# exanauts/SqpSolver.jl

Hardware: AMD Instinct MI355X
Metric: QP subproblems/sec on batched ACOPF; fp64 KKT LDL^T TFLOPS vs MFMA peak (higher is better)
Workload: dtype f64

## Files before the change

### sqpsolver.jl_amd/csrc/mfront.hip

```cpp
#include "ctx.hpp"
#include "dev_util.hpp"
#include "mf_dev.hpp"
#include <cstdlib>
#include <mutex>

namespace sqphip {

#ifdef SQPHIP_MF_TRACE
__device__ long long g_mf_trace[1 << 16][8];
#define MF_TR(i) if (inst == 0 && threadIdx.x == 0 && s < (1 << 16)) g_mf_trace[s][i] = (long long)wall_clock64();
__device__ long long g_mf_trace2[1 << 12][16];
#define MF_TRW(i) if (W == 0 && trs >= 0 && trs < (1 << 12) && lane == 0) g_mf_trace2[trs][i] = (long long)clock64();
__device__ long long g_mf_trace3[1 << 12][16];
#define MF_TRS(i) if (inst == 0 && tid == 0 && s < (1 << 12)) g_mf_trace3[s][i] = (long long)clock64();
#define MF_TR2S(a, b) if (inst == 0 && lane == 0 && j < 64 && wave < 2) g_mf_trace3[(do_fwd ? 64 : 0) + j][wave == 0 ? (a) : (b)] = (long long)clock64();
#define MF_TR2W(c) if (trj >= 0 && lane == 0) g_mf_trace3[trj][c] = (long long)clock64();
#define MF_TRSP(c) if (inst == 0 && cand == 0 && tid == 0 && k < 64) g_mf_trace3[128 + k][c] = (long long)wall_clock64();
#else
#define MF_TR(i)
#define MF_TRW(i)
#define MF_TRS(i)
#define MF_TR2S(a, b)
#define MF_TR2W(c)
#define MF_TRSP(c)
// ... 333 lines not shown
                    acc[q] = __builtin_amdgcn_mfma_f64_16x16x4f64(a, b, acc[q], 0, 0, 0);
                }
        }
    }
    __syncthreads();
    MF_TR(4)
    double *dinv = mf_dinv(d, inst, cand) + f0, *vv = mf_vv(d, inst, cand) + f0;
#pragma unroll
    for (int q = 0; q < MAXT; ++q) {
        if (ti_[q] < 0) continue;
#pragma unroll
        for (int rr = 0; rr < 4; ++rr) {
            const int col = 16 * tj_[q] + l4 + 4 * rr, row = 16 * ti_[q] + l15;
            const double v = acc[q][rr];
            if (col < nc) {
                if (row > col && row < fs) G[(long)col * ld + row] = v * dl[col];
                else if (row == fs && with_rhs) vv[col] = v * dl[col];
            } else if (col < fs && row >= col && row <= fs) G[(long)col * ld + row] = v;
        }
    }
    for (int k = tid; k < nc; k += NT) dinv[k] = dl[k];
    MF_TR(5)
}

struct MfBlk4 { double i0, i1, i2, i3, m10, m20, m21, m30, m31, m32; };

__device__ __forceinline__ MfBlk4 mf_ldl4(double a00, double a10, double a11, double a20, double a21, double a22, double a30,
                                           double a31, double a32, double a33, int bw)
{
    double i1 = 0.0, i2 = 0.0, i3 = 0.0, l21 = 0.0, l31 = 0.0, l32 = 0.0;
    const double i0 = mf_rcp(a00);
    const double l10 = a10 * i0, l20 = a20 * i0, l30 = a30 * i0;
#if SQPHIP_MF_LDL4_FAST
    {
        const double p11 = a10 * a10, p21 = a10 * a20, p22 = a20 * a20, p31 = a10 * a30, p32 = a20 * a30, p33 = a30 * a30;
        a11 = fma(-p11, i0, a11); a21 = fma(-p21, i0, a21); a22 = fma(-p22, i0, a22); a31 = fma(-p31, i0, a31); a32 = fma(-p32, i0, a32); a33 = fma(-p33, i0, a33);
    }
    if (bw > 1) {
        i1 = mf_rcp(a11); l21 = a21 * i1; l31 = a31 * i1;
        const double q22 = a21 * a21, q32 = a21 * a31, q33 = a31 * a31;
        a22 = fma(-q22, i1, a22); a32 = fma(-q32, i1, a32); a33 = fma(-q33, i1, a33);
    }
    if (bw > 2) { i2 = mf_rcp(a22); l32 = a32 * i2; a33 = fma(-(a32 * a32), i2, a33); }
#else
    a11 -= l10 * a10; a21 -= l10 * a20; a22 -= l20 * a20; a31 -= l10 * a30; a32 -= l20 * a30; a33 -= l30 * a30;
    if (bw > 1) { i1 = mf_rcp(a11); l21 = a21 * i1; l31 = a31 * i1; a22 -= l21 * a21; a32 -= l21 * a31; a33 -= l31 * a31; }
    if (bw > 2) { i2 = mf_rcp(a22); l32 = a32 * i2; a33 -= l32 * a32; }
#endif
    if (bw > 3) i3 = mf_rcp(a33);
    MfBlk4 B;
    B.i0 = i0; B.i1 = i1; B.i2 = i2; B.i3 = i3;
    B.m10 = -l10; B.m21 = -l21; B.m32 = -l32;
    B.m20 = -(l20 + l21 * B.m10);
    B.m31 = -(l31 + l32 * B.m21);
    B.m30 = -(l30 + l31 * B.m10 + l32 * B.m20);
    return B;
}

struct MfLaneSel { double s0, s1, s2, s3; };
__device__ __forceinline__ MfLaneSel mf_lane_sel(int l4)
{
    return {l4 == 0 ? 1.0 : 0.0, l4 == 1 ? 1.0 : 0.0, l4 == 2 ? 1.0 : 0.0, l4 == 3 ? 1.0 : 0.0};
}
__device__ __forceinline__ double mf_sel_ic(const MfLaneSel &S, const MfBlk4 &B)
{
    return fma(S.s3, B.i3, fma(S.s2, B.i2, fma(S.s1, B.i1, S.s0 * B.i0)));
}
__device__ __forceinline__ double mf_apply4(double x, int l15, const MfLaneSel &S, const MfBlk4 &B)
{
    const MfRows V = mf_rows3(x, l15);
    const double v0 = V.r0, v1 = V.r1, v2 = V.r2;
    const double c0 = fma(S.s3, B.m30, fma(S.s2, B.m20, S.s1 * B.m10));
    const double c1 = fma(S.s3, B.m31, S.s2 * B.m21);
    const double c2 = S.s3 * B.m32;
    return fma(c2, v2, fma(c1, v1, fma(c0, v0, x)));
}

__device__ __forceinline__ void wave_sync_lds()
{
    __builtin_amdgcn_fence(__ATOMIC_ACQ_REL, "wavefront");
    __builtin_amdgcn_wave_barrier();
}

__host__ __device__ constexpr int mf_front_lds_doubles(int T, int NW, bool ldsimg)
{
    const int R = 16 * T, u = (ldsimg ? R * R : 0) > 16 * R ? R * R : 16 * R;
    return u + 256 + 40 + R + 64 * NW;
}

template <int T, int NW, int W> struct MfTileSet {
    static constexpr int NROWS = W < T ? (T - W + NW - 1) / NW : 0;
    static constexpr int NTILES = NROWS > 0 ? NROWS * (2 * W + (NROWS - 1) * NW + 2) / 2 : 1;
};

template <int T, int NW, int W> struct MfAcc { d4 v[MfTileSet<T, NW, W>::NTILES]; };

template <int T, int NW, int W, bool LDSIMG>
__device__ __forceinline__ void mf_front_load(MfAcc<T, NW, W> &A, const double *F, int LD, int fs, int lane)
{
    auto &acc = A.v;
    constexpr int NROWS = MfTileSet<T, NW, W>::NROWS;
    const int l15 = lane & 15, l4 = lane >> 4;
    int o = 0;
#pragma unroll
    for (int s = 0; s < NROWS; ++s) {
        const int ti = W + s * NW;
#pragma unroll
        for (int tj = 0; tj <= ti; ++tj)
#pragma unroll
            for (int rr = 0; rr < 4; ++rr) {
                const int col = 16 * tj + l4 + 4 * rr, row = 16 * ti + l15;
                const bool in = LDSIMG || (row <= fs && col < fs);
                acc[o + tj][rr] = in ? F[col * LD + row] : 0.0;
            }
        o += ti + 1;
    }
}

__device__ __forceinline__ void lds_barrier()
{
    asm volatile("s_waitcnt lgkmcnt(0)\n\ts_barrier" ::: "memory");
}
template <bool LDSBAR> __device__ __forceinline__ void mf_elim_barrier() { if constexpr (LDSBAR) lds_barrier(); else __syncthreads(); }

template <int T, int NW, int W, bool LDSIMG>
__device__ __forceinline__ void mf_front_store_col(const MfAcc<T, NW, W> &A, int tk, double *G, int ld, int fs, int nc, int with_rhs,
                                                   const double *lds, double *vv, int lane)
{
    const auto &acc = A.v;
    constexpr int R = 16 * T;
    constexpr int U = (LDSIMG ? R * R : 0) > 16 * R ? R * R : 16 * R;
    constexpr int NROWS = MfTileSet<T, NW, W>::NROWS;
    const double *dl = lds + U + 256 + 40;
    const int l15 = lane & 15, l4 = lane >> 4;
    int o = 0;
#pragma unroll
    for (int s = 0; s < NROWS; ++s) {
        const int ti = W + s * NW;
        if (ti >= tk) {
            const bool inside = ti > tk && 16 * ti + 15 < fs;
            if (inside && 16 * tk + 15 < nc) {
#pragma unroll
                for (int rr = 0; rr < 4; ++rr) {
                    const int col = 16 * tk + l4 + 4 * rr;
                    G[(long)col * ld + 16 * ti + l15] = acc[o + tk][rr] * dl[col];
                }
            } else {
#pragma unroll
                for (int rr = 0; rr < 4; ++rr) {
                    const int col = 16 * tk + l4 + 4 * rr, row = 16 * ti + l15;
                    const double v = acc[o + tk][rr];
                    if (col < nc) {
                        if (row > col && row < fs) G[(long)col * ld + row] = v * dl[col];
                        else if (row == fs && with_rhs) vv[col] = v * dl[col];
                    }
                }
            }
        }
        o += ti + 1;
    }
}

template <int T, int NW, int W, bool LDSIMG, bool LDSBAR = false, bool EARLY = false>
__device__ __forceinline__ void mf_front_elim(MfAcc<T, NW, W> &A, int nc, double *lds, int lane, int trs, double *G = nullptr, int ld = 0,
                                              int fs = 0, int with_rhs = 0, double *vv = nullptr)
{
    auto &acc = A.v;
    constexpr int R = 16 * T;
    constexpr int U = (LDSIMG ? R * R : 0) > 16 * R ? R * R : 16 * R;
    constexpr int NROWS = MfTileSet<T, NW, W>::NROWS;
    double *Lp = lds, *dtile = lds + U, *rec = dtile + 256, *dl = rec + 40, *dsc = dl + R + 64 * W;
    const int l15 = lane & 15, l4 = lane >> 4;
    const MfLaneSel LS = mf_lane_sel(l4);
#pragma unroll
    for (int tk = 0; tk < T; ++tk) {
        if (16 * tk >= nc) break;
        if (tk == 1) { MF_TRW(9) }
        const int live = nc - 16 * tk;
        if (tk % NW == W) {
            constexpr int dummy = 0; (void)dummy;
            const int sd = (tk - W) / NW;
            const int od = sd * (2 * W + (sd - 1) * NW + 2) / 2 + tk;
            d4 dt = acc[od];
            d4 ls = {0.0, 0.0, 0.0, 0.0};
#pragma unroll
            for (int sub = 0; sub < 4; ++sub) {
                if (4 * sub >= live) break;
                const int bw = live - 4 * sub < 4 ? live - 4 * sub : 4, b0 = 4 * sub;
                const double dv = dt[sub];
#if SQPHIP_MF_SHFL
                dsc[lane] = dv;
                wave_sync_lds();
                if (tk == 0 && sub == 0) { MF_TRW(11) }
                const double a00 = dsc[b0], a10 = dsc[b0 + 1], a11 = dsc[b0 + 17], a20 = dsc[b0 + 2], a21 = dsc[b0 + 18],
                             a22 = dsc[b0 + 34], a30 = dsc[b0 + 3], a31 = dsc[b0 + 19], a32 = dsc[b0 + 35], a33 = dsc[b0 + 51];
                wave_sync_lds();
#else
                if (tk == 0 && sub == 0) { MF_TRW(11) }
                const double a00 = mf_readlane(dv, b0), a10 = mf_readlane(dv, b0 + 1), a11 = mf_readlane(dv, b0 + 17),
                             a20 = mf_readlane(dv, b0 + 2), a21 = mf_readlane(dv, b0 + 18), a22 = mf_readlane(dv, b0 + 34),
                             a30 = mf_readlane(dv, b0 + 3), a31 = mf_readlane(dv, b0 + 19), a32 = mf_readlane(dv, b0 + 35),
                             a33 = mf_readlane(dv, b0 + 51);
#endif
#ifdef SQPHIP_MF_TRACE
                if (tk == 0 && sub == 0) { asm volatile("s_waitcnt lgkmcnt(0)" ::: "memory"); MF_TRW(12) }
#endif
                const MfBlk4 B = mf_ldl4(a00, a10, a11, a20, a21, a22, a30, a31, a32, a33, bw);
#ifdef SQPHIP_MF_TRACE
                if (tk == 0 && sub == 0) { double tdep = B.m30; asm volatile("v_mov_b64 %0, %0" : "+v"(tdep)); MF_TRW(13) }
#endif
                const double x = mf_apply4(dv, l15, LS, B);
                const double ic = mf_sel_ic(LS, B);
                dt[sub] = x;
                ls[sub] = x * ic;
#ifdef SQPHIP_MF_TRACE
                if (tk == 0 && sub == 0) { double tdep = ls[sub]; asm volatile("v_mov_b64 %0, %0" : "+v"(tdep)); MF_TRW(14) }
#endif
                dt = __builtin_amdgcn_mfma_f64_16x16x4f64(l15 >= b0 + 4 ? -ls[sub] : 0.0, x, dt, 0, 0, 0);
#ifdef SQPHIP_MF_TRACE
                if (tk == 0 && sub == 0) { double tdep = dt[1]; asm volatile("v_mov_b64 %0, %0" : "+v"(tdep)); MF_TRW(15) }
#endif
                if (lane == 0) {
                    double *o = rec + 10 * sub;
                    o[0] = B.i0; o[1] = B.i1; o[2] = B.i2; o[3] = B.i3; o[4] = B.m10; o[5] = B.m20; o[6] = B.m21; o[7] = B.m30;
                    o[8] = B.m31; o[9] = B.m32;
                }
                if (l15 == 0 && l4 < bw) dl[16 * tk + b0 + l4] = ic;
            }
#pragma unroll
            for (int sub = 0; sub < 4; ++sub) dtile[64 * sub + lane] = ls[sub];
            acc[od] = dt;
        }
        if (tk == 0) { MF_TRW(3) }
        mf_elim_barrier<LDSBAR || EARLY>();
        if (tk == 0) { MF_TRW(4) }
        {
            int o = 0;
#pragma unroll
            for (int s = 0; s < NROWS; ++s) {
                const int ti = W + s * NW;
                if (ti > tk) {
                    d4 pt = acc[o + tk];
#pragma unroll
                    for (int sub = 0; sub < 4; ++sub) {
                        if (4 * sub >= live) break;
                        const double *q = rec + 10 * sub;
                        MfBlk4 B;
                        B.i0 = q[0]; B.i1 = q[1]; B.i2 = q[2]; B.i3 = q[3]; B.m10 = q[4]; B.m20 = q[5]; B.m21 = q[6]; B.m30 = q[7];
                        B.m31 = q[8]; B.m32 = q[9];
                        const double x = mf_apply4(pt[sub], l15, LS, B);
                        const double ic = mf_sel_ic(LS, B);
                        pt[sub] = x;
                        Lp[(4 * sub + l4) * R + 16 * ti + l15] = x * ic;
                        if (sub < 3) pt = __builtin_amdgcn_mfma_f64_16x16x4f64(l15 >= 4 * sub + 4 ? -dtile[64 * sub + lane] : 0.0, x, pt, 0, 0, 0);
                    }
                    acc[o + tk] = pt;
                }
                o += ti + 1;
            }
        }
        if (tk == 0) { MF_TRW(5) }
        mf_elim_barrier<LDSBAR || EARLY>();
        if (tk == 0) { MF_TRW(6) }
        {
            int o = 0;
#pragma unroll
            for (int s = 0; s < NROWS; ++s) {
                const int ti = W + s * NW;
                if (ti > tk) {
                    const d4 xr = acc[o + tk];
#pragma unroll
                    for (int tj = tk + 1; tj <= ti; ++tj)
#pragma unroll
                        for (int sub = 0; sub < 4; ++sub) {
                            if (4 * sub >= live) break;
                            acc[o + tj] = __builtin_amdgcn_mfma_f64_16x16x4f64(-Lp[(4 * sub + l4) * R + 16 * tj + l15], xr[sub], acc[o + tj], 0, 0, 0);
                        }
                }
                o += ti + 1;
            }
        }
        if constexpr (EARLY) mf_front_store_col<T, NW, W, LDSIMG>(A, tk, G, ld, fs, nc, with_rhs, lds, vv, lane);
    }
}

template <int T, int NW, int W, bool LDSIMG, bool EARLY = false>
__device__ __forceinline__ void mf_front_store(const MfAcc<T, NW, W> &A, double *G, int ld, int fs, int nc,
                                               int with_rhs, double *CB, int ldcb, const double *lds, double *dinv, double *vv, int lane)
{
    const auto &acc = A.v;
    constexpr int R = 16 * T;
    constexpr int U = (LDSIMG ? R * R : 0) > 16 * R ? R * R : 16 * R;
    constexpr int NROWS = MfTileSet<T, NW, W>::NROWS;
    const double *dl = lds + U + 256 + 40;
    const int l15 = lane & 15, l4 = lane >> 4;
    int o = 0;
#pragma unroll
    for (int s = 0; s < NROWS; ++s) {
        const int ti = W + s * NW;
#pragma unroll
        for (int tj = 0; tj <= ti; ++tj) {
            const bool inside = ti > tj && 16 * ti + 15 < fs;
            if (inside && 16 * tj + 15 < nc) {
                if constexpr (!EARLY) {
#pragma unroll
                    for (int rr = 0; rr < 4; ++rr) {
                        const int col = 16 * tj + l4 + 4 * rr;
                        G[(long)col * ld + 16 * ti + l15] = acc[o + tj][rr] * dl[col];
                    }
                }
            } else if (inside && 16 * tj >= nc) {
#pragma unroll
                for (int rr = 0; rr < 4; ++rr) CB[(long)(16 * tj + l4 + 4 * rr) * ldcb + 16 * ti + l15] = acc[o + tj][rr];
            } else {
#pragma unroll
                for (int rr = 0; rr < 4; ++rr) {
                    const int col = 16 * tj + l4 + 4 * rr, row = 16 * ti + l15;
                    const double v = acc[o + tj][rr];
                    if (col < nc) {
                        if constexpr (!EARLY) {
                            if (row > col && row < fs) G[(long)col * ld + row] = v * dl[col];
                            else if (row == fs && with_rhs) vv[col] = v * dl[col];
                        }
                    } else if (col < fs && row >= col && row <= fs) CB[(long)col * ldcb + row] = v;
                }
            }
        }
        o += ti + 1;
    }
    if (W == 0) for (int k = lane; k < nc; k += 64) dinv[k] = dl[k];
}

template <int T, int NW, int W, bool LDSIMG, bool LDSBAR = false, bool EARLY = false>
__device__ __forceinline__ void mf_front_wave(const double *F, int LD, double *G, int ld, int fs, int nc, int with_rhs,
                                              double *lds, double *dinv, double *vv, int lane, int trs, double *CB, int ldcb)
{
    MF_TRW(0)
    MfAcc<T, NW, W> acc;
    mf_front_load<T, NW, W, LDSIMG>(acc, F, LD, fs, lane);
    MF_TRW(1)
    mf_elim_barrier<LDSBAR>();
    MF_TRW(2)
    mf_front_elim<T, NW, W, LDSIMG, LDSBAR, EARLY>(acc, nc, lds, lane, trs, G, ld, fs, with_rhs, vv);
    MF_TRW(7)
    mf_elim_barrier<LDSBAR || EARLY>();
    MF_TRW(8)
    mf_front_store<T, NW, W, LDSIMG, EARLY>(acc, G, ld, fs, nc, with_rhs, CB, ldcb, lds, dinv, vv, lane);
    MF_TRW(10)
}

template <int T, int NW, int W, bool LDSIMG>
__device__ __forceinline__ void mf_front_dispatch(int wave, const double *F, int LD, double *G, int ld, int fs, int nc,
                                                  int with_rhs, double *lds, double *dinv, double *vv, int lane, int trs)
{
    if (wave == W) mf_front_wave<T, NW, W, LDSIMG, false, (SQPHIP_MF_EARLY_STORE != 0 && T >= 5)>(F, LD, G, ld, fs, nc, with_rhs, lds, dinv, vv, lane, trs, G, ld);
    else if constexpr (W + 1 < NW) mf_front_dispatch<T, NW, W + 1, LDSIMG>(wave, F, LD, G, ld, fs, nc, with_rhs, lds, dinv, vv, lane, trs);
}

template <int T, int NW, bool LDSIMG>
__global__ __launch_bounds__(64 * NW) void k_mf_front(DV d, int sbegin, int want, int with_rhs)
{
    constexpr int NT = 64 * NW, R = 16 * T;
    int inst, cand;
    if (!mf_candidate(d, want, inst, cand)) return;
    const MfDev &M = d.mf;
    const int s = M.sched[sbegin + blockIdx.x];
    const MfFrontDesc Fd = M.desc[s];
    const int nc = Fd.nc, nr = Fd.nr, fs = nc + nr, ld = fs + 1, f0 = Fd.first;
    const double *arena = mf_arena(d, inst, cand);
    double *G = mf_arena(d, inst, cand) + Fd.off;
    extern __shared__ double mf_lds[];
    double *F = LDSIMG ? mf_lds : G;
    const int LD = LDSIMG ? R : ld;
    const int tid = threadIdx.x;
    MF_TR(0)
    constexpr int PV = 4, PE = 8;
    int vrc[PV]; double vval[PV]; int ew[PE], eb[PE], ee[PE]; double ea[PE];
    {
        const double *vals = mf_vals(d, inst, cand);
#pragma unroll
        for (int k = 0; k < PV; ++k) {
            const int e = Fd.asm_begin + tid + k * NT;
            vrc[k] = -1; vval[k] = 0.0;
            if (e < Fd.asm_end) { vrc[k] = M.dest_rc[e]; vval[k] = vals[e]; }
        }
#pragma unroll
        for (int k = 0; k < PE; ++k) {
            const int t = Fd.ea_begin + tid + k * NT;
            ew[k] = -1; eb[k] = 0; ee[k] = 0; ea[k] = 0.0;
            if (t < Fd.ea_end) { const MfGather g = M.ea_ent[t]; ew[k] = g.where; eb[k] = g.src_begin; ee[k] = g.src_end; ea[k] = arena[g.src0]; }
        }
    }
    double brhs = 0.0;
    if (with_rhs && tid < nc) brhs = d.xv[(long)inst * d.Fpad + f0 + tid];
    if (LDSIMG) for (int e = tid; e < R * R; e += NT) F[e] = 0.0;
    else for (int e = tid; e < ld * fs; e += NT) F[e] = 0.0;
    __syncthreads();
    MF_TR(1)
    {
        const double *vals = mf_vals(d, inst, cand);
#pragma unroll
        for (int k = 0; k < PV; ++k) if (vrc[k] >= 0) F[(vrc[k] >> 16) * LD + (vrc[k] & 0xffff)] = vval[k];
        for (int e = Fd.asm_begin + tid + PV * NT; e < Fd.asm_end; e += NT) {
            const int rc = M.dest_rc[e];
            F[(rc >> 16) * LD + (rc & 0xffff)] = vals[e];
        }
        if (with_rhs) {
            if (tid < nc) F[tid * LD + fs] = brhs;
            const double *b = d.xv + (long)inst * d.Fpad + f0;
            for (int j = tid + NT; j < nc; j += NT) F[j * LD + fs] = b[j];
        }
    }
    __syncthreads();
    MF_TR(2)
#pragma unroll
    for (int k = 0; k < PE; ++k)
        if (ew[k] >= 0) {
            double a = ea[k];
            for (int q = eb[k] + 1; q < ee[k]; ++q) a += arena[M.ea_src[q]];
            F[(ew[k] >> 16) * LD + (ew[k] & 0xffff)] += a;
        }
    for (int t = Fd.ea_begin + tid + PE * NT; t < Fd.ea_end; t += NT) {
        const MfGather g = M.ea_ent[t];
        double a = arena[g.src0];
        for (int q = g.src_begin + 1; q < g.src_end; ++q) a += arena[M.ea_src[q]];
        const int rc = g.where;
        F[(rc >> 16) * LD + (rc & 0xffff)] += a;
    }
    __syncthreads();
    MF_TR(3)
    const int wave = __builtin_amdgcn_readfirstlane(tid >> 6);
    mf_front_dispatch<T, NW, 0, LDSIMG>(wave, F, LD, G, ld, fs, nc, with_rhs, mf_lds, mf_dinv(d, inst, cand) + f0,
                                        mf_vv(d, inst, cand) + f0, tid & 63, inst == 0 ? s : -1);
    MF_TR(4)
    MF_TR(5)
}

constexpr int MF_SP_NW = 8, MF_SP_NT = 64 * MF_SP_NW, MF_SP_PV = 3, MF_SP_PE = 6;
struct MfSpinePre { int vrc[MF_SP_PV]; double vval[MF_SP_PV]; int ew[MF_SP_PE], eb[MF_SP_PE], ee[MF_SP_PE], es[MF_SP_PE]; double ea[MF_SP_PE]; double brhs; };

template <int T, int W>
__device__ __forceinline__ void mf_spine_dispatch_w(int wave, double *lds, double *G, int ld, int fs, int nc, int with_rhs, double *dinv,
                                                    double *vv, int lane, double *CB, int ldcb)
{
    if (wave == W) mf_front_wave<T, MF_SP_NW, W, true, true>(lds, 16 * T, G, ld, fs, nc, with_rhs, lds, dinv, vv, lane, -1, CB, ldcb);
    else if constexpr (W + 1 < MF_SP_NW) mf_spine_dispatch_w<T, W + 1>(wave, lds, G, ld, fs, nc, with_rhs, dinv, vv, lane, CB, ldcb);
}
template <int T>
__device__ __forceinline__ void mf_spine_dispatch_t(int Tf, int wave, double *lds, double *G, int ld, int fs, int nc, int with_rhs, double *dinv,
                                                    double *vv, int lane, double *CB, int ldcb)
{
    if (Tf == T) mf_spine_dispatch_w<T, 0>(wave, lds, G, ld, fs, nc, with_rhs, dinv, vv, lane, CB, ldcb);
    else if constexpr (T < 8) mf_spine_dispatch_t<T + 1>(Tf, wave, lds, G, ld, fs, nc, with_rhs, dinv, vv, lane, CB, ldcb);
}

__global__ __launch_bounds__(MF_SP_NT) void k_mf_spine(DV d, int want, int with_rhs)
{
    constexpr int NT = MF_SP_NT, PV = MF_SP_PV, PE = MF_SP_PE;
    int inst, cand;
    if (!mf_candidate(d, want, inst, cand)) return;
    const MfDev &M = d.mf;
    extern __shared__ double mf_lds[];
    const int tid = threadIdx.x, lane = tid & 63, wave = __builtin_amdgcn_readfirstlane(tid >> 6);
    double *arena = mf_arena(d, inst, cand);
    const double *vals = mf_vals(d, inst, cand);
    const double *xv = d.xv + (long)inst * d.Fpad;
    double *dinv = mf_dinv(d, inst, cand), *vv = mf_vv(d, inst, cand);
    double *stage = mf_lds + mf_front_lds_doubles(M.sp_T, MF_SP_NW, true);
    int *relmap = reinterpret_cast<int *>(stage + M.sp_stage);
    const int n = M.sp_n;
    auto rec = [&](int k) {
        MfSpineFront R;
        const int *g = reinterpret_cast<const int *>(M.sp_fr + k);
        int *w = reinterpret_cast<int *>(&R);
#pragma unroll
        for (int q = 0; q < 12; ++q) w[q] = __builtin_amdgcn_readfirstlane(g[q]);
        R.pad0 = R.pad1 = R.pad2 = R.pad3 = 0;
        return R;
    };
    auto issue1 = [&](const MfSpineFront &R, MfSpinePre &P) {
#pragma unroll
        for (int k = 0; k < PV; ++k) {
            const int e = R.asm_begin + tid + k * NT;
            P.vrc[k] = -1; P.vval[k] = 0.0;
            if (e < R.asm_end) { P.vrc[k] = M.dest_rc[e]; P.vval[k] = vals[e]; }
        }
#pragma unroll
        for (int k = 0; k < PE; ++k) {
            const int t = R.ea_begin + tid + k * NT;
            P.ew[k] = -1; P.eb[k] = 0; P.ee[k] = 0; P.es[k] = 0; P.ea[k] = 0.0;
            if (t < R.ea_end) { const MfGather g = M.sp_ent[t]; P.ew[k] = g.where; P.eb[k] = g.src_begin; P.ee[k] = g.src_end; P.es[k] = g.src0; }
        }
        P.brhs = (with_rhs && tid < R.nc) ? xv[R.first + tid] : 0.0;
    };
    auto issue2 = [&](MfSpinePre &P) {
#pragma unroll
        for (int k = 0; k < PE; ++k) if (P.ew[k] >= 0) P.ea[k] = arena[P.es[k]];
    };
    auto begin_image = [&](const MfSpineFront &R, const MfSpinePre &P, int slot) {
        const int Rn = 16 * R.T;
        for (int e = tid; e < Rn * Rn; e += NT) mf_lds[e] = 0.0;
        if (R.handoff && tid <= R.nr) relmap[136 * slot + tid] = M.sp_rel[R.rel + tid];
        lds_barrier();
#pragma unroll
        for (int k = 0; k < PE; ++k)
            if (P.ew[k] >= 0) {
                double a = P.ea[k];
                for (int q = P.eb[k] + 1; q < P.ee[k]; ++q) a += arena[M.sp_src[q]];
                mf_lds[(P.ew[k] >> 16) * Rn + (P.ew[k] & 0xffff)] += a;
            }
        for (int t = R.ea_begin + tid + PE * NT; t < R.ea_end; t += NT) {
            const MfGather g = M.sp_ent[t];
            double a = arena[g.src0];
            for (int q = g.src_begin + 1; q < g.src_end; ++q) a += arena[M.sp_src[q]];
            mf_lds[(g.where >> 16) * Rn + (g.where & 0xffff)] += a;
// ... 851 lines not shown
        __syncthreads();
    }
}

template <bool HASBIG>
__global__ __launch_bounds__(256, HASBIG ? 4 : 5) void k_mf_bwd2(DV d, int ibegin, int want, int wimg, int also)
{
    const int inst = blockIdx.y;
    const int ph = d.phase[inst];
    if (ph != want && ph != also) return;
    extern __shared__ double mf_lds[];
    const MfDev &M = d.mf;
    const int4 it = reinterpret_cast<const int4 *>(M.sol_items)[ibegin + blockIdx.x];
    const int tid = threadIdx.x, lane = tid & 63, wave = __builtin_amdgcn_readfirstlane(tid >> 6);
    const bool big = HASBIG && it.y == -2;
    const int s = big ? it.x : (wave == 0 ? it.x : (wave == 1 ? it.y : (wave == 2 ? it.z : it.w)));
    if (s < 0) return;
    const MfFrontDesc Fd = M.desc[s];
    const int nc = Fd.nc, nr = Fd.nr, fs = nc + nr, ld = fs + 1, f0 = Fd.first, ll = fs | 1;
    const int cand = d.ist[inst].sel;
    const double *G = mf_arena(d, inst, cand) + Fd.off;
    double *xg = d.xv + (long)inst * d.Fpad;
    const double *vv = mf_vv(d, inst, cand) + f0;
    const int *rows = M.rows + Fd.rowptr;
    double *Bf = (big ? mf_lds : mf_lds + wave * (64 + wimg)) + (big ? 128 : 64);
    const int i0 = lane, i1 = lane + 64;
    if (!big || wave == 0) {
        const int q0 = i0 < nr ? rows[i0] : -1, q1 = (big && i1 < nr) ? rows[i1] : -1;
        double t0 = i0 < nc ? vv[i0] : 0.0, t1 = (big && i1 < nc) ? vv[i1] : 0.0;
        if (!big) mf_img_load<1, 24, false>(G, ld, nc, fs, Bf, ll, 0, lane);
        else mf_img_load<4, 14, true>(G, ld, nc, fs, Bf, ll, 0, lane);
        const double xr0 = q0 >= 0 ? xg[q0] : 0.0, xr1 = q1 >= 0 ? xg[q1] : 0.0;
        if (big) __syncthreads(); else wave_sync();
        if (nc <= 64) mf_chain_bwd<false>(Bf, ll, nc, nr, lane, xr0, xr1, t0, t1);
        else mf_chain_bwd<true>(Bf, ll, nc, nr, lane, xr0, xr1, t0, t1);
        if (i0 < nc) xg[f0 + i0] = t0;
        if (big && i1 < nc) xg[f0 + i1] = t1;
    } else {
        mf_img_load<4, 14, true>(G, ld, nc, fs, Bf, ll, wave, lane);
        __syncthreads();
    }
}

const char *const mf_kernel_names[] = {
    "k_mf_values", "k_mf_factor<256, true>", "k_mf_factor2<1, 3, true>", "k_mf_factor2<2, 5, true>", "k_mf_factor2<4, 4, true>",
    "k_mf_factor2<4, 9, false>", "k_mf_factor2<8, 12, false>",
    "k_mf_front<1, 1, true>", "k_mf_front<2, 1, true>", "k_mf_front<3, 1, true>", "k_mf_front<4, 2, true>", "k_mf_front<4, 4, true>",
    "k_mf_front<5, 2, true>", "k_mf_front<5, 4, true>",
    "k_mf_front<6, 4, false>", "k_mf_front<6, 4, true>", "k_mf_front<6, 8, true>",
    "k_mf_front<7, 4, false>", "k_mf_front<7, 4, true>", "k_mf_front<7, 8, true>",
    "k_mf_front<8, 4, false>", "k_mf_front<8, 4, true>", "k_mf_front<8, 8, true>",
    "k_mf_front<9, 8, false>", "k_mf_front<10, 8, false>", "k_mf_front<11, 8, false>", "k_mf_front<12, 8, false>",
    "k_mf_spine", "k_mf_solve_inst<16>", "k_mf_fwd", "k_mf_fwd2<false>", "k_mf_fwd2<true>", "k_mf_solve_top", "k_mf_solve_top2",
    "k_mf_bwd", "k_mf_bwd2<false>", "k_mf_bwd2<true>", "k_inertia" };
static_assert(sizeof(mf_kernel_names) / sizeof(mf_kernel_names[0]) == MFK_COUNT, "a name per MfKernel entry");
static constexpr int mf_front_kid(int T, int NW, bool IMG)
{
    return T >= 1 && T <= 3 ? (NW == 1 && IMG ? MFK_FRONT_1 + T - 1 : -1)
         : T <= 5 ? ((NW == 2 || NW == 4) && IMG ? MFK_FRONT_4_2 + 2 * (T - 4) + (NW == 4) : -1)
         : T <= 8 ? (NW == 4 ? MFK_FRONT_6_4 + 3 * (T - 6) + (IMG ? 1 : 0) : NW == 8 && IMG ? MFK_FRONT_6_4 + 3 * (T - 6) + 2 : -1)
         : T <= 12 ? (NW == 8 && !IMG ? MFK_FRONT_9 + T - 9 : -1) : -1;
}
static constexpr int mf_factor2_kid(int NW, int MAXT, bool IMG)
{
    return NW == 1 && MAXT == 3 && IMG ? MFK_F2_1_3 : NW == 2 && MAXT == 5 && IMG ? MFK_F2_2_5 : NW == 4 && MAXT == 4 && IMG ? MFK_F2_4_4
         : NW == 4 && MAXT == 9 && !IMG ? MFK_F2_4_9 : NW == 8 && MAXT == 12 && !IMG ? MFK_F2_8_12 : -1;
}

static int mf_generic_solves()
{
    static const int g = getenv("SQPHIP_MF_GENERIC") ? atoi(getenv("SQPHIP_MF_GENERIC")) : 0;
    return g;
}

void mf_device_setup(Ctx &C)
{
    static std::mutex mu;
    std::lock_guard<std::mutex> lk(mu);
    bool ok = true;
    auto big = [&](const void *f) { ok &= hipFuncSetAttribute(f, hipFuncAttributeMaxDynamicSharedMemorySize, 160 * 1024) == hipSuccess; };
    big(reinterpret_cast<const void *>(k_mf_front<6, 4, true>)); big(reinterpret_cast<const void *>(k_mf_front<7, 4, true>));
    big(reinterpret_cast<const void *>(k_mf_front<8, 4, true>)); big(reinterpret_cast<const void *>(k_mf_front<6, 8, true>));
    big(reinterpret_cast<const void *>(k_mf_front<7, 8, true>)); big(reinterpret_cast<const void *>(k_mf_front<8, 8, true>));
    big(reinterpret_cast<const void *>(k_mf_fwd2<true>)); big(reinterpret_cast<const void *>(k_mf_bwd2<true>));
    big(reinterpret_cast<const void *>(k_mf_fwd2<false>)); big(reinterpret_cast<const void *>(k_mf_bwd2<false>));
    big(reinterpret_cast<const void *>(k_mf_solve_top2));
    big(reinterpret_cast<const void *>(k_mf_spine));
    (void)hipGetLastError();
    C.mf_big_lds = ok;
}

void mf_values(Ctx &C, int want)
{
    const DV &d = C.d;
    hipStream_t s = C.stream;
    const int nb = d.mf.fronts1 && d.spec_mode != 0 ? 2 * d.B : d.B;
    const bool serial = d.mf.nvblk == 0 || (getenv("SQPHIP_MF_VALUES_SERIAL") && atoi(getenv("SQPHIP_MF_VALUES_SERIAL")) != 0);
    C.tm.open(s); C.mf_census[MFK_VALUES]++;
    if (serial) hipLaunchKernelGGL(k_mf_values_serial, dim3((d.mf.nnzK + 255) / 256, nb), dim3(256), 0, s, d, want);
    else hipLaunchKernelGGL(k_mf_values, dim3(d.mf.nvblk, nb), dim3(MF_VBLK_ITEMS), 0, s, d, want);
    C.tm.close(KC_VALUES, s);
}

static inline bool mf_launch_narrow(const MfLaunch &L, int narrow_level) { return L.level >= narrow_level; }
bool mf_same_selection(const MfLaunch &a, const MfLaunch &b, int narrow_level)
{
    return a.tiles == b.tiles && a.small == b.small &&
           (a.tiles >= 4 || mf_launch_narrow(a, narrow_level) == mf_launch_narrow(b, narrow_level));
}

void mf_factor(Ctx &C, int want, bool with_rhs, bool values_done)
{
    const DV &d = C.d;
    hipStream_t s = C.stream;
    static const bool v1 = getenv("SQPHIP_MF_V1") != nullptr;
    const int wr = (int)with_rhs;
    const int nb = d.mf.fronts1 && d.spec_mode != 0 ? 2 * d.B : d.B;
    if (!v1 && !values_done) mf_values(C, want);
    const bool stat = !(getenv("SQPHIP_MF_STATIC") && atoi(getenv("SQPHIP_MF_STATIC")) == 0);
    const bool packed = !(getenv("SQPHIP_MF_F2_PACKED") && atoi(getenv("SQPHIP_MF_F2_PACKED")) == 0);
    const bool spine = !v1 && d.mf.sp_n > 0 && C.mf_big_lds;
    int li = 0, cls_open = -1;
    for (const MfLaunch &L : C.mfp().fac) {
        if (spine && li++ >= C.mfp().fac_below) break;
        const int cls = mf_launch_narrow(L, C.mfp().narrow_level) ? KC_FRONTS_TOP : KC_FRONTS_LOW;
        if (cls != cls_open) { if (cls_open >= 0) C.tm.close(cls_open, s); C.tm.open(s); cls_open = cls; }
        const dim3 grid(L.count, nb);
        const int T = L.tiles;
        if (v1 || T > 13) { C.mf_census[MFK_FACTOR_R1]++; hipLaunchKernelGGL((k_mf_factor<256, true>), grid, dim3(256), 0, s, d, L.begin, want, wr); continue; }
#define MF_GENERIC(NW, MAXT, IMG) do { constexpr int kid_ = mf_factor2_kid(NW, MAXT, IMG); static_assert(kid_ >= 0, "census: no counter"); C.mf_census[kid_]++; \
        if (IMG && packed) hipLaunchKernelGGL((k_mf_factor2<NW, MAXT, IMG, IMG>), grid, dim3(64 * NW), 8 * mf_factor2_lds_doubles(T, IMG, true), s, d, L.begin, want, wr, T); \
        else hipLaunchKernelGGL((k_mf_factor2<NW, MAXT, IMG, false>), grid, dim3(64 * NW), 8 * mf_factor2_lds_doubles(T, IMG, false), s, d, L.begin, want, wr, T); } while (0)
#define MF_STATIC(TT, NW, IMG) do { constexpr int kid_ = mf_front_kid(TT, NW, IMG); static_assert(kid_ >= 0, "census: no counter"); C.mf_census[kid_]++; hipLaunchKernelGGL((k_mf_front<TT, NW, IMG>), grid, dim3(64 * NW), 8 * (size_t)mf_front_lds_doubles(TT, NW, IMG), s, d, L.begin, want, wr); } while (0)
        const int stat_min = getenv("SQPHIP_MF_STATIC_MIN") ? atoi(getenv("SQPHIP_MF_STATIC_MIN")) : (L.small && mf_launch_narrow(L, C.mfp().narrow_level) ? 1 : 4);
        const bool nw8 = !(getenv("SQPHIP_MF_NW8") && atoi(getenv("SQPHIP_MF_NW8")) == 0);
        const int nw4 = L.small ? (getenv("SQPHIP_MF_NW4") ? atoi(getenv("SQPHIP_MF_NW4")) : 3) : 0;
        const bool big_img = C.mf_big_lds && !(getenv("SQPHIP_MF_BIG_LDSIMG") && atoi(getenv("SQPHIP_MF_BIG_LDSIMG")) == 0);
        static const int stat_max = getenv("SQPHIP_MF_STATIC_MAX") ? atoi(getenv("SQPHIP_MF_STATIC_MAX")) : 12;
        if (!stat || T > stat_max || T > 12 || T < stat_min) {
            if (T <= 2) MF_GENERIC(1, 3, true);
            else if (T <= 4) MF_GENERIC(2, 5, true);
            else if (T <= 5) MF_GENERIC(4, 4, true);
            else if (T <= 8) MF_GENERIC(4, 9, false);
            else MF_GENERIC(8, 12, false);
            continue;
        }
        switch (T) {
        case 1: MF_STATIC(1, 1, true); break;
        case 2: MF_STATIC(2, 1, true); break;
        case 3: MF_STATIC(3, 1, true); break;
        case 4: if (nw4 & 1) MF_STATIC(4, 4, true); else MF_STATIC(4, 2, true); break;
        case 5: if (nw4 & 2) MF_STATIC(5, 4, true); else MF_STATIC(5, 2, true); break;
        case 6: if (big_img && L.small) { if (nw8) MF_STATIC(6, 8, true); else MF_STATIC(6, 4, true); } else MF_STATIC(6, 4, false); break;
        case 7: if (big_img && L.small) { if (nw8) MF_STATIC(7, 8, true); else MF_STATIC(7, 4, true); } else MF_STATIC(7, 4, false); break;
        case 8: if (big_img && L.small) { if (nw8) MF_STATIC(8, 8, true); else MF_STATIC(8, 4, true); } else MF_STATIC(8, 4, false); break;
        case 9: MF_STATIC(9, 8, false); break;
        case 10: MF_STATIC(10, 8, false); break;
        case 11: MF_STATIC(11, 8, false); break;
        default: MF_STATIC(12, 8, false); break;
        }
#undef MF_GENERIC
#undef MF_STATIC
    }
    if (cls_open >= 0) C.tm.close(cls_open, s);
    if (spine) { C.tm.open(s); C.mf_census[MFK_SPINE]++; hipLaunchKernelGGL(k_mf_spine, dim3(1, nb), dim3(MF_SP_NT), (size_t)C.mfp().spine_lds_bytes, s, d, want, wr); C.tm.close(KC_FRONTS_TOP, s); }
    C.mf_factor_launches += spine ? (long)C.mfp().fac_below + 1 : (long)C.mfp().fac.size();
}

bool mf_solve_tests_inertia(const Ctx &C)
{
    static const bool off = getenv("SQPHIP_MF_INERTIA_KERNEL") != nullptr;
    return !off && C.d.sparse && C.d.mf.top_n > 0 && !mf_generic_solves() && !(C.d.B >= (getenv("SQPHIP_MF_INST_SOLVE_MIN") ? atoi(getenv("SQPHIP_MF_INST_SOLVE_MIN")) : (1 << 30)));
}

void mf_solve(Ctx &C, int want, bool skip_fwd, bool inertia, int also)
{
    const DV &d = C.d;
    hipStream_t s = C.stream;
    const int generic = mf_generic_solves();
    static const int inst_min = getenv("SQPHIP_MF_INST_SOLVE_MIN") ? atoi(getenv("SQPHIP_MF_INST_SOLVE_MIN")) : (1 << 30);
    if (d.B >= inst_min && d.mf.max_front * 8 * 16 <= 64 * 1024) {
        C.mf_census[MFK_SOLVE_INST]++;
        hipLaunchKernelGGL(k_mf_solve_inst<16>, dim3(d.B), dim3(1024), (size_t)d.mf.max_front * 8 * 16, s, d, want, skip_fwd ? 0 : 1, generic);
        return;
    }
    const bool lvl2 = !(getenv("SQPHIP_MF_LEVEL2") && atoi(getenv("SQPHIP_MF_LEVEL2")) == 0);
    if (!C.mf_big_lds) throw std::string("sqphip: the solve kernels could not be granted 160 KB of dynamic LDS on this device (mf_device_setup)");
    if (also >= 0 && !(skip_fwd && d.mf.top_n > 0 && !generic && d.B < inst_min)) throw std::string("sqphip: mf_solve: a second phase needs the streamed top behind a fused forward pass");
    const int fwant = also >= 0 ? also : want;
    const bool run_fwd = !skip_fwd || also >= 0;
    if (run_fwd && !C.mfp().fwd.empty()) C.tm.open(s);
    if (run_fwd)
        for (const MfLaunch &L : C.mfp().fwd) {
            C.mf_census[lvl2 && !generic && L.wimg >= 0 ? (L.hasbig ? MFK_FWD2_BIG : MFK_FWD2) : MFK_FWD]++;
            if (lvl2 && !generic && L.wimg >= 0) {
                if (L.hasbig) hipLaunchKernelGGL(k_mf_fwd2<true>, dim3(L.count, d.B), dim3(256), L.lds2, s, d, L.begin, fwant, L.wimg);
                else hipLaunchKernelGGL(k_mf_fwd2<false>, dim3(L.count, d.B), dim3(256), L.lds2, s, d, L.begin, fwant, L.wimg);
            }
            else hipLaunchKernelGGL(k_mf_fwd, dim3(L.count, d.B), dim3(256), L.lds_bytes, s, d, L.begin, fwant, generic, L.tiles, L.cls, L.lds_bytes / 8 - L.cls);
        }
    if (run_fwd && !C.mfp().fwd.empty()) C.tm.close(KC_SOLVE_LEVELS, s);
    const bool has_top = (d.mf.top_n > 0 && !generic) || C.mfp().top.count > 0;
    if (has_top) C.tm.open(s);
    if (d.mf.top_n > 0 && !generic) {
        const size_t lds = (size_t)C.mfp().top2_lds_bytes;
        C.mf_census[MFK_SOLVE_TOP2]++;
        const char *ser = getenv("SQPHIP_INERTIA_SERIAL");
        hipLaunchKernelGGL(k_mf_solve_top2, dim3(d.B), dim3(256), lds, s, d, want, skip_fwd ? 0 : 1, inertia ? (ser && atoi(ser) ? 2 : 1) : 0, also);
    } else if (const MfLaunch &T = C.mfp().top; T.count > 0) {
        C.mf_census[MFK_SOLVE_TOP]++;
        hipLaunchKernelGGL(k_mf_solve_top, dim3(d.B), dim3(256), T.lds_bytes, s, d, T.begin, T.count, want, skip_fwd ? 0 : 1, generic,
                           T.tiles, T.cls, T.lds_bytes / 8 - T.cls);
    }
    if (has_top) C.tm.close(KC_SOLVE_TOP, s);
    if (!C.mfp().bwd.empty()) C.tm.open(s);
    for (const MfLaunch &L : C.mfp().bwd) {
// ... 12 lines not shown
```

Measured before the change: 10530.

## Use packed lower-triangular tile layout for the static front LDS image

```diff
diff --git a/sqpsolver.jl_amd/csrc/mfront.hip b/sqpsolver.jl_amd/csrc/mfront.hip
--- a/sqpsolver.jl_amd/csrc/mfront.hip
+++ b/sqpsolver.jl_amd/csrc/mfront.hip
@@ -439,10 +439,18 @@
     __builtin_amdgcn_wave_barrier();
 }
 
-__host__ __device__ constexpr int mf_front_lds_doubles(int T, int NW, bool ldsimg)
-{
-    const int R = 16 * T, u = (ldsimg ? R * R : 0) > 16 * R ? R * R : 16 * R;
-    return u + 256 + 40 + R + 64 * NW;
+__host__ __device__ constexpr int mf_front_img_doubles(int T, bool ldsimg, bool packed)
+{
+    const int R = 16 * T, img = !ldsimg ? 0 : packed ? 128 * T * (T + 1) : R * R;
+    return img > 16 * R ? img : 16 * R;
+}
+__host__ __device__ constexpr bool mf_front_img_holds_rows(int T) { return 128 * T * (T + 1) >= 16 * 16 * T; }
+static_assert(mf_front_img_holds_rows(1) && mf_front_img_holds_rows(2) && mf_front_img_holds_rows(3) && mf_front_img_holds_rows(4) &&
+              mf_front_img_holds_rows(5) && mf_front_img_holds_rows(6) && mf_front_img_holds_rows(7) && mf_front_img_holds_rows(8),
+              "packed image: 128 T (T + 1) >= 16 R for every T with an LDS image (equality at T = 1)");
+__host__ __device__ constexpr int mf_front_lds_doubles(int T, int NW, bool ldsimg, bool packed = false)
+{
+    return mf_front_img_doubles(T, ldsimg, packed) + 256 + 40 + 16 * T + 64 * NW;
 }
 
 template <int T, int NW, int W> struct MfTileSet {
@@ -452,9 +460,10 @@
 
 template <int T, int NW, int W> struct MfAcc { d4 v[MfTileSet<T, NW, W>::NTILES]; };
 
-template <int T, int NW, int W, bool LDSIMG>
+template <int T, int NW, int W, bool LDSIMG, bool PACKED = false>
 __device__ __forceinline__ void mf_front_load(MfAcc<T, NW, W> &A, const double *F, int LD, int fs, int lane)
 {
+    static_assert(LDSIMG || !PACKED, "the packed layout is that of the LDS image");
     auto &acc = A.v;
     constexpr int NROWS = MfTileSet<T, NW, W>::NROWS;
     const int l15 = lane & 15, l4 = lane >> 4;
@@ -468,7 +477,7 @@
             for (int rr = 0; rr < 4; ++rr) {
                 const int col = 16 * tj + l4 + 4 * rr, row = 16 * ti + l15;
                 const bool in = LDSIMG || (row <= fs && col < fs);
-                acc[o + tj][rr] = in ? F[col * LD + row] : 0.0;
+                acc[o + tj][rr] = in ? F[PACKED ? 256 * (ti * (ti + 1) / 2 + tj) + 64 * rr + lane : col * LD + row] : 0.0;
             }
         o += ti + 1;
     }
@@ -480,13 +489,12 @@
 }
 template <bool LDSBAR> __device__ __forceinline__ void mf_elim_barrier() { if constexpr (LDSBAR) lds_barrier(); else __syncthreads(); }
 
-template <int T, int NW, int W, bool LDSIMG>
+template <int T, int NW, int W, bool LDSIMG, bool PACKED = false>
 __device__ __forceinline__ void mf_front_store_col(const MfAcc<T, NW, W> &A, int tk, double *G, int ld, int fs, int nc, int with_rhs,
                                                    const double *lds, double *vv, int lane)
 {
     const auto &acc = A.v;
-    constexpr int R = 16 * T;
-    constexpr int U = (LDSIMG ? R * R : 0) > 16 * R ? R * R : 16 * R;
+    constexpr int U = mf_front_img_doubles(T, LDSIMG, PACKED);
     constexpr int NROWS = MfTileSet<T, NW, W>::NROWS;
     const double *dl = lds + U + 256 + 40;
     const int l15 = lane & 15, l4 = lane >> 4;
@@ -518,13 +526,13 @@
     }
 }
 
-template <int T, int NW, int W, bool LDSIMG, bool LDSBAR = false, bool EARLY = false>
+template <int T, int NW, int W, bool LDSIMG, bool LDSBAR = false, bool EARLY = false, bool PACKED = false>
 __device__ __forceinline__ void mf_front_elim(MfAcc<T, NW, W> &A, int nc, double *lds, int lane, int trs, double *G = nullptr, int ld = 0,
                                               int fs = 0, int with_rhs = 0, double *vv = nullptr)
 {
     auto &acc = A.v;
     constexpr int R = 16 * T;
-    constexpr int U = (LDSIMG ? R * R : 0) > 16 * R ? R * R : 16 * R;
+    constexpr int U = mf_front_img_doubles(T, LDSIMG, PACKED);
     constexpr int NROWS = MfTileSet<T, NW, W>::NROWS;
     double *Lp = lds, *dtile = lds + U, *rec = dtile + 256, *dl = rec + 40, *dsc = dl + R + 64 * W;
     const int l15 = lane & 15, l4 = lane >> 4;
@@ -637,17 +645,16 @@
                 o += ti + 1;
             }
         }
-        if constexpr (EARLY) mf_front_store_col<T, NW, W, LDSIMG>(A, tk, G, ld, fs, nc, with_rhs, lds, vv, lane);
-    }
-}
-
-template <int T, int NW, int W, bool LDSIMG, bool EARLY = false>
+        if constexpr (EARLY) mf_front_store_col<T, NW, W, LDSIMG, PACKED>(A, tk, G, ld, fs, nc, with_rhs, lds, vv, lane);
+    }
+}
+
+template <int T, int NW, int W, bool LDSIMG, bool EARLY = false, bool PACKED = false>
 __device__ __forceinline__ void mf_front_store(const MfAcc<T, NW, W> &A, double *G, int ld, int fs, int nc,
                                                int with_rhs, double *CB, int ldcb, const double *lds, double *dinv, double *vv, int lane)
 {
     const auto &acc = A.v;
-    constexpr int R = 16 * T;
-    constexpr int U = (LDSIMG ? R * R : 0) > 16 * R ? R * R : 16 * R;
+    constexpr int U = mf_front_img_doubles(T, LDSIMG, PACKED);
     constexpr int NROWS = MfTileSet<T, NW, W>::NROWS;
     const double *dl = lds + U + 256 + 40;
     const int l15 = lane & 15, l4 = lane >> 4;
@@ -688,35 +695,38 @@
     if (W == 0) for (int k = lane; k < nc; k += 64) dinv[k] = dl[k];
 }
 
-template <int T, int NW, int W, bool LDSIMG, bool LDSBAR = false, bool EARLY = false>
+template <int T, int NW, int W, bool LDSIMG, bool LDSBAR = false, bool EARLY = false, bool PACKED = false>
 __device__ __forceinline__ void mf_front_wave(const double *F, int LD, double *G, int ld, int fs, int nc, int with_rhs,
                                               double *lds, double *dinv, double *vv, int lane, int trs, double *CB, int ldcb)
 {
     MF_TRW(0)
     MfAcc<T, NW, W> acc;
-    mf_front_load<T, NW, W, LDSIMG>(acc, F, LD, fs, lane);
+    mf_front_load<T, NW, W, LDSIMG, PACKED>(acc, F, LD, fs, lane);
     MF_TRW(1)
     mf_elim_barrier<LDSBAR>();
     MF_TRW(2)
-    mf_front_elim<T, NW, W, LDSIMG, LDSBAR, EARLY>(acc, nc, lds, lane, trs, G, ld, fs, with_rhs, vv);
+    mf_front_elim<T, NW, W, LDSIMG, LDSBAR, EARLY, PACKED>(acc, nc, lds, lane, trs, G, ld, fs, with_rhs, vv);
     MF_TRW(7)
     mf_elim_barrier<LDSBAR || EARLY>();
     MF_TRW(8)
-    mf_front_store<T, NW, W, LDSIMG, EARLY>(acc, G, ld, fs, nc, with_rhs, CB, ldcb, lds, dinv, vv, lane);
+    mf_front_store<T, NW, W, LDSIMG, EARLY, PACKED>(acc, G, ld, fs, nc, with_rhs, CB, ldcb, lds, dinv, vv, lane);
     MF_TRW(10)
 }
 
-template <int T, int NW, int W, bool LDSIMG>
+template <int T, int NW, int W, bool LDSIMG, bool PACKED>
 __device__ __forceinline__ void mf_front_dispatch(int wave, const double *F, int LD, double *G, int ld, int fs, int nc,
                                                   int with_rhs, double *lds, double *dinv, double *vv, int lane, int trs)
 {
-    if (wave == W) mf_front_wave<T, NW, W, LDSIMG, false, (SQPHIP_MF_EARLY_STORE != 0 && T >= 5)>(F, LD, G, ld, fs, nc, with_rhs, lds, dinv, vv, lane, trs, G, ld);
-    else if constexpr (W + 1 < NW) mf_front_dispatch<T, NW, W + 1, LDSIMG>(wave, F, LD, G, ld, fs, nc, with_rhs, lds, dinv, vv, lane, trs);
-}
-
-template <int T, int NW, bool LDSIMG>
+    if (wave == W) mf_front_wave<T, NW, W, LDSIMG, false, (SQPHIP_MF_EARLY_STORE != 0 && T >= 5), PACKED>(F, LD, G, ld, fs, nc, with_rhs, lds, dinv, vv, lane, trs, G, ld);
+    else if constexpr (W + 1 < NW) mf_front_dispatch<T, NW, W + 1, LDSIMG, PACKED>(wave, F, LD, G, ld, fs, nc, with_rhs, lds, dinv, vv, lane, trs);
+}
+
+template <bool PACKED> __device__ __forceinline__ int mf_front_at(int row, int col, int LD) { return PACKED ? mf_pk(row, col) : col * LD + row; }
+
+template <int T, int NW, bool LDSIMG, bool PACKED = false>
 __global__ __launch_bounds__(64 * NW) void k_mf_front(DV d, int sbegin, int want, int with_rhs)
 {
+    static_assert(LDSIMG || !PACKED, "the packed layout is that of the LDS image");
     constexpr int NT = 64 * NW, R = 16 * T;
     int inst, cand;
     if (!mf_candidate(d, want, inst, cand)) return;
@@ -750,22 +760,23 @@
     }
     double brhs = 0.0;
     if (with_rhs && tid < nc) brhs = d.xv[(long)inst * d.Fpad + f0 + tid];
-    if (LDSIMG) for (int e = tid; e < R * R; e += NT) F[e] = 0.0;
+    if (PACKED) for (int e = tid; e < 128 * T * (T + 1); e += NT) F[e] = 0.0;
+    else if (LDSIMG) for (int e = tid; e < R * R; e += NT) F[e] = 0.0;
     else for (int e = tid; e < ld * fs; e += NT) F[e] = 0.0;
     __syncthreads();
     MF_TR(1)
     {
         const double *vals = mf_vals(d, inst, cand);
 #pragma unroll
-        for (int k = 0; k < PV; ++k) if (vrc[k] >= 0) F[(vrc[k] >> 16) * LD + (vrc[k] & 0xffff)] = vval[k];
+        for (int k = 0; k < PV; ++k) if (vrc[k] >= 0) F[mf_front_at<PACKED>(vrc[k] & 0xffff, vrc[k] >> 16, LD)] = vval[k];
         for (int e = Fd.asm_begin + tid + PV * NT; e < Fd.asm_end; e += NT) {
             const int rc = M.dest_rc[e];
-            F[(rc >> 16) * LD + (rc & 0xffff)] = vals[e];
+            F[mf_front_at<PACKED>(rc & 0xffff, rc >> 16, LD)] = vals[e];
         }
         if (with_rhs) {
-            if (tid < nc) F[tid * LD + fs] = brhs;
+            if (tid < nc) F[mf_front_at<PACKED>(fs, tid, LD)] = brhs;
             const double *b = d.xv + (long)inst * d.Fpad + f0;
-            for (int j = tid + NT; j < nc; j += NT) F[j * LD + fs] = b[j];
+            for (int j = tid + NT; j < nc; j += NT) F[mf_front_at<PACKED>(fs, j, LD)] = b[j];
         }
     }
     __syncthreads();
@@ -775,19 +786,19 @@
         if (ew[k] >= 0) {
             double a = ea[k];
             for (int q = eb[k] + 1; q < ee[k]; ++q) a += arena[M.ea_src[q]];
-            F[(ew[k] >> 16) * LD + (ew[k] & 0xffff)] += a;
+            F[mf_front_at<PACKED>(ew[k] & 0xffff, ew[k] >> 16, LD)] += a;
         }
     for (int t = Fd.ea_begin + tid + PE * NT; t < Fd.ea_end; t += NT) {
         const MfGather g = M.ea_ent[t];
         double a = arena[g.src0];
         for (int q = g.src_begin + 1; q < g.src_end; ++q) a += arena[M.ea_src[q]];
         const int rc = g.where;
-        F[(rc >> 16) * LD + (rc & 0xffff)] += a;
+        F[mf_front_at<PACKED>(rc & 0xffff, rc >> 16, LD)] += a;
     }
     __syncthreads();
     MF_TR(3)
     const int wave = __builtin_amdgcn_readfirstlane(tid >> 6);
-    mf_front_dispatch<T, NW, 0, LDSIMG>(wave, F, LD, G, ld, fs, nc, with_rhs, mf_lds, mf_dinv(d, inst, cand) + f0,
+    mf_front_dispatch<T, NW, 0, LDSIMG, PACKED>(wave, F, LD, G, ld, fs, nc, with_rhs, mf_lds, mf_dinv(d, inst, cand) + f0,
                                         mf_vv(d, inst, cand) + f0, tid & 63, inst == 0 ? s : -1);
     MF_TR(4)
     MF_TR(5)
@@ -1805,6 +1816,9 @@
     big(reinterpret_cast<const void *>(k_mf_front<6, 4, true>)); big(reinterpret_cast<const void *>(k_mf_front<7, 4, true>));
     big(reinterpret_cast<const void *>(k_mf_front<8, 4, true>)); big(reinterpret_cast<const void *>(k_mf_front<6, 8, true>));
     big(reinterpret_cast<const void *>(k_mf_front<7, 8, true>)); big(reinterpret_cast<const void *>(k_mf_front<8, 8, true>));
+    big(reinterpret_cast<const void *>(k_mf_front<6, 4, true, true>)); big(reinterpret_cast<const void *>(k_mf_front<7, 4, true, true>));
+    big(reinterpret_cast<const void *>(k_mf_front<8, 4, true, true>)); big(reinterpret_cast<const void *>(k_mf_front<6, 8, true, true>));
+    big(reinterpret_cast<const void *>(k_mf_front<7, 8, true, true>)); big(reinterpret_cast<const void *>(k_mf_front<8, 8, true, true>));
     big(reinterpret_cast<const void *>(k_mf_fwd2<true>)); big(reinterpret_cast<const void *>(k_mf_bwd2<true>));
     big(reinterpret_cast<const void *>(k_mf_fwd2<false>)); big(reinterpret_cast<const void *>(k_mf_bwd2<false>));
     big(reinterpret_cast<const void *>(k_mf_solve_top2));
@@ -1842,6 +1856,7 @@
     if (!v1 && !values_done) mf_values(C, want);
     const bool stat = !(getenv("SQPHIP_MF_STATIC") && atoi(getenv("SQPHIP_MF_STATIC")) == 0);
     const bool packed = !(getenv("SQPHIP_MF_F2_PACKED") && atoi(getenv("SQPHIP_MF_F2_PACKED")) == 0);
+    const bool fpacked = !(getenv("SQPHIP_MF_FRONT_PACKED") && atoi(getenv("SQPHIP_MF_FRONT_PACKED")) == 0);
     const bool spine = !v1 && d.mf.sp_n > 0 && C.mf_big_lds;
     int li = 0, cls_open = -1;
     for (const MfLaunch &L : C.mfp().fac) {
@@ -1854,7 +1869,9 @@
 #define MF_GENERIC(NW, MAXT, IMG) do { constexpr int kid_ = mf_factor2_kid(NW, MAXT, IMG); static_assert(kid_ >= 0, "census: no counter"); C.mf_census[kid_]++; \
         if (IMG && packed) hipLaunchKernelGGL((k_mf_factor2<NW, MAXT, IMG, IMG>), grid, dim3(64 * NW), 8 * mf_factor2_lds_doubles(T, IMG, true), s, d, L.begin, want, wr, T); \
         else hipLaunchKernelGGL((k_mf_factor2<NW, MAXT, IMG, false>), grid, dim3(64 * NW), 8 * mf_factor2_lds_doubles(T, IMG, false), s, d, L.begin, want, wr, T); } while (0)
-#define MF_STATIC(TT, NW, IMG) do { constexpr int kid_ = mf_front_kid(TT, NW, IMG); static_assert(kid_ >= 0, "census: no counter"); C.mf_census[kid_]++; hipLaunchKernelGGL((k_mf_front<TT, NW, IMG>), grid, dim3(64 * NW), 8 * (size_t)mf_front_lds_doubles(TT, NW, IMG), s, d, L.begin, want, wr); } while (0)
+#define MF_STATIC(TT, NW, IMG) do { constexpr int kid_ = mf_front_kid(TT, NW, IMG); static_assert(kid_ >= 0, "census: no counter"); C.mf_census[kid_]++; \
+        if (IMG && fpacked) hipLaunchKernelGGL((k_mf_front<TT, NW, IMG, IMG>), grid, dim3(64 * NW), 8 * (size_t)mf_front_lds_doubles(TT, NW, IMG, IMG), s, d, L.begin, want, wr); \
+        else hipLaunchKernelGGL((k_mf_front<TT, NW, IMG, false>), grid, dim3(64 * NW), 8 * (size_t)mf_front_lds_doubles(TT, NW, IMG, false), s, d, L.begin, want, wr); } while (0)
         const int stat_min = getenv("SQPHIP_MF_STATIC_MIN") ? atoi(getenv("SQPHIP_MF_STATIC_MIN")) : (L.small && mf_launch_narrow(L, C.mfp().narrow_level) ? 1 : 4);
         const bool nw8 = !(getenv("SQPHIP_MF_NW8") && atoi(getenv("SQPHIP_MF_NW8")) == 0);
         const int nw4 = L.small ? (getenv("SQPHIP_MF_NW4") ? atoi(getenv("SQPHIP_MF_NW4")) : 3) : 0;
```

After: 10940, median of 6. 1.04x the previous value.
